# uthree/ALiVE-VC

Measured on AMD Instinct MI355X. Metric: VC frames/sec + RTF @24kHz, 1M-vec library; 1/2/4/8 MI355X, higher is better.
Workload: dtype decoder fp16 GEMMs / fp32 acc; encoders 22-bit fp16 split; kNN exact fp32 top-k via fp6 MFMA candidates (certified); f32 MFMA small convs; f64 phase scan

## Files before the change

### alive-vc_amd/csrc/conv.hip

```cpp
#include "conv_epilogue.h"
#include "planes_layout.h"

namespace {

constexpr int BK = 16;
constexpr int A_LD = BK + 4;

template <int BM, int BN, int WM, int WN, bool UPV = false, bool YPL = false>
__global__ __launch_bounds__(256) void conv_gemm_kernel(AliveConv p, unsigned kw_magic, unsigned kw_shift, float film_ratio) {
    constexpr int TM = BM / WM, TN = BN / WN;
    constexpr int MR = TM / 16, NR = TN / 16;
    constexpr int B_LD = BN + 4;
    constexpr int ROWS_PER_PASS = 256 / BN;
    constexpr int EPT = BK / ROWS_PER_PASS;
    constexpr int A_VEC = (BM * 4 + 255) / 256;
    static_assert(WM * WN == 4, "4 waves");
    static_assert(256 % BN == 0 || BN == 256, "BN");

    __shared__ __attribute__((aligned(16))) float As[2][BM][A_LD];
    __shared__ __attribute__((aligned(16))) float Bs[2][BK][B_LD];

    const int tid = threadIdx.x;
    const int lane = tid & 63;
    const int wid = tid >> 6;
// ... 117 lines not shown
                if (p.up == 4) {
                    if (row < p.Co) *(f32x4*)(p.Y + ((size_t)n * Cq + (row >> 2)) * Lout + (size_t)t * 4) = acc[m][nn];
                } else {
#pragma unroll
                    for (int h = 0; h < 2; ++h)
                        if (row + 2 * h < p.Co) {
                            f32x2 v = {acc[m][nn][2 * h], acc[m][nn][2 * h + 1]};
                            *(f32x2*)(p.Y + ((size_t)n * Cq + (row >> 1) + h) * Lout + (size_t)t * 2) = v;
                        }
                }
            }
        }
        return;
    }
#pragma unroll
    for (int nn = 0; nn < NR; ++nn) {
        const int t = t0 + wn * TN + nn * 16 + lr;
        if (t >= p.Tout) continue;
        Lerp lp;
        if (p.Z != nullptr) lp = lerp_coord(t, film_ratio, p.Lf);
#pragma unroll
        for (int m = 0; m < MR; ++m) {
#pragma unroll
            for (int r = 0; r < 4; ++r) {
                const int row_local = wm * TM + m * 16 + lq * 4 + r;
                if (m0 + row_local >= p.Co) continue;
                conv_epilogue_store<false>(p, n, m0 + row_local, row_local, t, acc[m][nn][r], lp, ft);
            }
        }
        if constexpr (YPL) {
            static_assert(!YPL || (MR % 2) == 0, "the plane image pairs the 16-row groups");
            const int c_pad = (p.Co + 31) & ~31;
            const int64_t cols_pad = (((int64_t)p.N * p.Tout + 127) / 128) * 128;
            unsigned short* Po = (unsigned short*)p.Yp;
            const bool odd = (lq & 1) != 0;
#pragma unroll
            for (int mp = 0; mp < MR; mp += 2) {
                const int rbase = m0 + wm * TM + mp * 16;
                if (rbase >= c_pad) continue;
                float qa[4], qb[4];
#pragma unroll
                for (int r = 0; r < 4; ++r) {
                    qa[r] = rbase + lq * 4 < p.Co ? acc[mp][nn][r] : 0.0f;
                    qb[r] = rbase + 16 + lq * 4 < p.Co ? acc[mp + 1][nn][r] : 0.0f;
                }
                const bool one_f16 = p.yp_planes == 1;
#pragma unroll
                for (int pl = 0; pl < 2; ++pl) {
                    if (pl == 1 && one_f16) break;
                    typedef __bf16 bf16x2_t __attribute__((ext_vector_type(2)));
                    auto pk = [one_f16](float a, float b) {
                        const bf16x2_t h = {(__bf16)a, (__bf16)b};
                        return one_f16 ? pack_f16x2(a, b) : __builtin_bit_cast(unsigned, h);
                    };
                    const unsigned a01 = pk(qa[0], qa[1]), a23 = pk(qa[2], qa[3]), b01 = pk(qb[0], qb[1]), b23 = pk(qb[2], qb[3]);
                    const unsigned rx = (unsigned)__shfl_xor((int)(odd ? a01 : b01), 16), ry = (unsigned)__shfl_xor((int)(odd ? a23 : b23), 16);
                    const u32x4 o = odd ? u32x4{rx, ry, b01, b23} : u32x4{a01, a23, rx, ry};
                    const int ch = rbase + (odd ? 16 + (lq - 1) * 4 : lq * 4);
                    *(u32x4*)(Po + planes_at(pl, (int64_t)n * p.Tout + t, ch, cols_pad, c_pad)) = o;
                    qa[0] -= __uint_as_float(a01 << 16); qa[1] -= __uint_as_float(a01 & 0xffff0000u);
                    qa[2] -= __uint_as_float(a23 << 16); qa[3] -= __uint_as_float(a23 & 0xffff0000u);
                    qb[0] -= __uint_as_float(b01 << 16); qb[1] -= __uint_as_float(b01 & 0xffff0000u);
                    qb[2] -= __uint_as_float(b23 << 16); qb[3] -= __uint_as_float(b23 & 0xffff0000u);
                }
            }
        }
    }
    if constexpr (YPL) {
        if (n == p.N - 1 && blockIdx.x == gridDim.x - 1) {
            const int c_pad = (p.Co + 31) & ~31;
            const int64_t cols = (int64_t)p.N * p.Tout, cols_pad = ((cols + 127) / 128) * 128;
            const int per_col = (p.yp_planes == 1 ? 1 : 2) * (c_pad / 4);
            unsigned short* Po = (unsigned short*)p.Yp;
            for (int i = threadIdx.x; i < (int)(cols_pad - cols) * per_col; i += 256) {
                const int c = i / per_col, w = i % per_col;
                *(uint2*)(Po + planes_at(w / (c_pad / 4), cols + c, (w % (c_pad / 4)) * 4, cols_pad, c_pad)) = make_uint2(0u, 0u);
            }
        }
    }
}

}

int alive_conv_split_launch(const AliveConv* d, float ratio, hipStream_t s);
bool alive_conv_skinny_try(const AliveConv* d, hipStream_t s, int* rc);

extern "C" int alive_conv1d(const AliveConv* d, void* stream) {
    ALIVE_CHECK_ARG(d && d->W && (d->X || d->Xp), "alive_conv1d: null W/X");
    ALIVE_CHECK_ARG(d->N > 0 && d->Ci > 0 && d->Co > 0 && d->Tin > 0 && d->Tout > 0, "alive_conv1d: bad sizes");
    ALIVE_CHECK_ARG(d->KW >= 1 && (d->KW <= 16 || d->Ci == 1) && d->stride >= 1 && d->dil >= 1 && d->up >= 1, "alive_conv1d: bad geometry");
    ALIVE_CHECK_ARG(d->precision >= 1 || (d->K_pad % 16 == 0 && d->K_pad >= d->Ci * d->KW), "alive_conv1d: K_pad %d for K %d", d->K_pad, d->Ci * d->KW);
    ALIVE_CHECK_ARG(d->precision >= 0 && d->precision <= 3, "alive_conv1d: precision");
    ALIVE_CHECK_ARG(d->Ci * d->KW < 32768, "alive_conv1d: K too large");
    ALIVE_CHECK_ARG(d->Y || d->Z || d->Zp, "alive_conv1d: no output");
    if (d->up > 1) {
        ALIVE_CHECK_ARG(d->Co % d->up == 0 && !d->residual && !d->skip && !d->Z && !d->Zp && d->Y, "alive_conv1d: transposed conv has a plain epilogue");
    }
    ALIVE_CHECK_ARG(d->yp_planes >= 0 && d->yp_planes <= 2, "alive_conv1d: yp_planes");
    if (d->Yp)
        ALIVE_CHECK_ARG(d->precision == 0 && d->Y && d->up == 1 && d->act == 0 && !d->post_add && !d->ch_scale && !d->residual && !d->skip && !d->Z &&
                        !d->Zp && d->Co > 16 && d->Co <= 64 && (d->Co & 3) == 0 && (((uintptr_t)d->Yp) & 15) == 0 && (int64_t)d->N * d->Tout >= 97,
                        "alive_conv1d: Yp (plane image of Y) needs the exact kernel's plain conv with 16 < Co <= 64, Co %% 4 == 0, more than 96 columns");
    ALIVE_CHECK_ARG(d->pad_mode >= 0 && d->pad_mode <= 2, "alive_conv1d: pad_mode");
    if (d->pad_mode != 0) ALIVE_CHECK_ARG(d->pad_left < d->Tin, "alive_conv1d: reflect pad %d needs Tin > pad (Tin %d)", d->pad_left, d->Tin);
    if (d->Z || d->Zp) ALIVE_CHECK_ARG(d->film && d->Lf > 0, "alive_conv1d: Z needs film");
    ALIVE_CHECK_ARG(d->film_ld != 0 || (d->film_t0 == 0 && d->film_f0 == 0), "alive_conv1d: film_t0 %d / film_f0 %d without a frame range (film_ld 0)",
                    d->film_t0, d->film_f0);
    if (d->precision == 3)
        ALIVE_CHECK_ARG((int64_t)d->N * d->Tout > 96, "alive_conv1d: precision 3 (plain fp16) is a batch form: more than 96 columns, got %lld",
                        (long long)d->N * d->Tout);
    if (d->Xp || d->Zp) ALIVE_CHECK_ARG(d->precision == 1 || d->precision == 3, "alive_conv1d: plane-packed operands need the split kernel (precision 1 or 3)");
    {
        int rc;
        if (d->film_ld == 0 && !d->Xp && !d->Zp && alive_conv_skinny_try(d, (hipStream_t)stream, &rc)) return rc;
    }
    if (d->precision >= 1)
        return alive_conv_split_launch(d, (d->Z || d->Zp) ? (float)(d->film_ld ? d->film_ld : d->Lf) / (float)d->Tout : 0.0f, (hipStream_t)stream);
    ALIVE_CHECK_ARG(d->film_ld == 0, "alive_conv1d: a film frame range needs the split kernel (precision 1 / 2)");
    const unsigned shift = d->KW < 4 ? 18u : d->KW < 8 ? 19u : 20u;
    const unsigned magic = d->Ci == 1 ? 0u : (unsigned)(((1u << shift) + d->KW - 1) / d->KW);
    const float ratio = d->Z ? (float)d->Lf / (float)d->Tout : 0.0f;
    hipStream_t s = (hipStream_t)stream;
    if (d->Co > 64) {
        dim3 g(cdiv(d->Tout, 128), cdiv(d->Co, 128), d->N);
        conv_gemm_kernel<128, 128, 2, 2><<<g, 256, 0, s>>>(*d, magic, shift, ratio);
    } else if (d->Co > 16) {
        dim3 g(cdiv(d->Tout, 128), cdiv(d->Co, 64), d->N);
        if (d->Yp) conv_gemm_kernel<64, 128, 1, 4, false, true><<<g, 256, 0, s>>>(*d, magic, shift, ratio);
        else conv_gemm_kernel<64, 128, 1, 4><<<g, 256, 0, s>>>(*d, magic, shift, ratio);
    } else {
        dim3 g(cdiv(d->Tout, 256), 1, d->N);
        if ((d->up == 2 || d->up == 4) && d->act == 0 && !d->post_add && !d->ch_scale)
            conv_gemm_kernel<16, 256, 1, 4, true><<<g, 256, 0, s>>>(*d, magic, shift, ratio);
        else
            conv_gemm_kernel<16, 256, 1, 4><<<g, 256, 0, s>>>(*d, magic, shift, ratio);
    }
    ALIVE_CHECK_LAUNCH("alive_conv1d");
    return ALIVE_OK;
}

ALIVE_F16_SAT_GETTER(alive_f16_sat_conv)
```

### alive-vc_amd/csrc/conv_split.hip

```cpp
#include "conv_epilogue.h"
#include "planes_layout.h"

namespace {

constexpr int BN = 128;
constexpr int BKC = 32;
constexpr int XROWS = 144;
constexpr int PITCH = 80;
constexpr int XPLANE = XROWS * PITCH;

typedef __bf16 bf16x2_t __attribute__((ext_vector_type(2)));

__device__ __forceinline__ bf16x8 lds_frag(const unsigned char* p) { return *(const bf16x8*)p; }

typedef const __attribute__((address_space(1))) void* gptr_t;
typedef __attribute__((address_space(3))) void* lptr_t;
constexpr int PROW = 64;

template <int BM, int NP, bool PLANES = false, bool W22 = false>
__global__ __launch_bounds__(256, 2) void conv_split_kernel(AliveConv p, float film_ratio) {
    static_assert(!W22 || BM == 128, "the 2 x 2 wave arrangement is the 128-row tile's");
    constexpr int NR = W22 ? 2 : (BM >= 128 ? 4 : 2);
    constexpr int MR = W22 ? 2 : 1;

// ... 302 lines not shown
            }
        } else if (upvec) {
            const int sh = __builtin_ctz((unsigned)p.up);
            const size_t Lout = (size_t)p.Tout * p.up;
#pragma unroll
            for (int g = tid; g < PR * (BN / 4); g += 256) {
                const int e = g * 4;
                const int co_l = e >> (7 + sh), rem = e & ((BN << sh) - 1);
                const int t_l = rem >> sh, j0 = rem & (p.up - 1);
                const int pr = (co_l << sh) + j0;
                const int row = m0 + ps * 64 + pr;
                const int t = t0 + t_l;
                if (row >= p.Co || t >= p.Tout) continue;
                f32x4 v;
#pragma unroll
                for (int q = 0; q < 4; ++q) {
                    float x = Ct[(pr + q) * CP + t_l];
                    if (p.act == 1) x = gelu_fast(x);
                    else if (p.act == 2) x = expf(x);
                    if (p.post_add != nullptr) x += p.post_add[row + q];
                    if (p.ch_scale != nullptr) x *= p.ch_scale[row + q];
                    v[q] = x;
                }
                *(f32x4*)(p.Y + ((size_t)n * (p.Co >> sh) + (row >> sh)) * Lout + ((size_t)t << sh) + j0) = v;
            }
        } else if (p.up > 1) {
            const unsigned inv_up = (unsigned)((0x100000000ull + (unsigned)p.up - 1) / (unsigned)p.up);
            const int R0 = m0 + ps * 64;
            const int c_first = (int)__umulhi((unsigned)R0, inv_up);
            int R1 = R0 + PR - 1;
            R1 = R1 < p.Co ? R1 : p.Co - 1;
            const int nch = (int)__umulhi((unsigned)R1, inv_up) - c_first + 1;
            const int per_ch = BN * p.up;
            const size_t Lout = (size_t)p.Tout * p.up;
            const int Cq = (int)__umulhi((unsigned)p.Co, inv_up);
#pragma unroll 1
            for (int ch = 0; ch < nch; ++ch) {
                const int co = c_first + ch;
                float* yrow = p.Y + ((size_t)n * Cq + co) * Lout + (size_t)t0 * p.up;
#pragma unroll 2
                for (int e = tid; e < per_ch; e += 256) {
                    const int t_l = (int)__umulhi((unsigned)e, inv_up), jj = e - t_l * p.up;
                    const int row = co * p.up + jj;
                    if (row < R0 || row > R1 || t0 + t_l >= p.Tout) continue;
                    float v = Ct[(row - R0) * CP + t_l];
                    if (p.act == 1) v = gelu_fast(v);
                    else if (p.act == 2) v = expf(v);
                    if (p.post_add != nullptr) v = v + p.post_add[row];
                    if (p.ch_scale != nullptr) v = v * p.ch_scale[row];
                    yrow[e] = v;
                }
            }
        } else {
#pragma unroll 1
            for (int g = tid; g < PR * BN; g += 256) {
                const int pr = g >> 7, c = g & 127;
                const int row = m0 + ps * 64 + pr;
                const int t = t0 + c;
                if (row >= p.Co || t >= p.Tout) continue;
                float v = Ct[pr * CP + c];
                if (p.act == 1) v = gelu_fast(v);
                else if (p.act == 2) v = expf(v);
                if (p.post_add != nullptr) v = v + p.post_add[row];
                if (p.ch_scale != nullptr) v = v * p.ch_scale[row];
                const size_t o = ((size_t)n * p.Co + row) * p.Tout + t;
                if (p.residual != nullptr) v = v + p.residual[o];
                if (p.skip != nullptr) v = v + p.skip[o];
                if (p.Y != nullptr) p.Y[o] = v;
                if (p.Z != nullptr) {
                    const float* fs = Ft + pr * 2 * FILM_NF - f_lo;
                    Lerp lp = lerp_coord(t + p.film_t0, film_ratio, p.Lf);
                    float sc = lerp_apply(lp, fs[lp.i0], fs[lp.i1]);
                    float sh = lerp_apply(lp, fs[FILM_NF + lp.i0], fs[FILM_NF + lp.i1]);
                    p.Z[o] = gelu_fast(v) * sc + sh;
                }
            }
        }
        __syncthreads();
    }
}

}

int alive_conv_split_launch(const AliveConv* d, float ratio, hipStream_t s) {
    ALIVE_CHECK_ARG(d->stride == 1, "alive_conv1d(split): stride must be 1");
    ALIVE_CHECK_ARG(d->Ci_pad % BKC == 0 && d->Ci_pad >= d->Ci, "alive_conv1d(split): Ci_pad %d for Ci %d", d->Ci_pad, d->Ci);
    ALIVE_CHECK_ARG(d->KW <= 8 && (d->KW - 1) * d->dil <= XROWS - BN, "alive_conv1d(split): halo (KW-1)*dil = %d exceeds %d",
                    (d->KW - 1) * d->dil, XROWS - BN);
    ALIVE_CHECK_ARG(d->pad_mode == 0 || d->pad_mode == 1, "alive_conv1d(split): pad_mode");
    ALIVE_CHECK_ARG(((((uintptr_t)d->Y) | ((uintptr_t)d->Z) | ((uintptr_t)d->residual) | ((uintptr_t)d->skip)) & 15) == 0,
                    "alive_conv1d(split): Y / Z / residual / skip must be 16-byte aligned");
    if (d->Z) {
        const double span = (double)(d->film_ld ? d->film_ld : d->Lf) / (double)d->Tout * BN + 3.0;
        ALIVE_CHECK_ARG(span <= FILM_NF, "alive_conv1d(split): FiLM second output needs Tout >= ~8 Lf (got Lf %d, Tout %d)", d->Lf, d->Tout);
    }
    ALIVE_CHECK_ARG(d->act >= 0 && d->act <= 2, "alive_conv1d(split): activation %d not available on the split kernel", d->act);
    if (d->Zp) {
        const double span = (double)(d->film_ld ? d->film_ld : d->Lf) / (double)d->Tout * BN + 3.0;
        ALIVE_CHECK_ARG(span <= FILM_NF && d->film, "alive_conv1d(split): plane second output needs FiLM rows and Tout >= ~8 Lf");
        ALIVE_CHECK_ARG(d->up == 1 && (d->Tout & 3) == 0 && d->Co % 64 == 0 && d->Co > 64 && (d->precision == 1 || d->precision == 3) &&
                        (((uintptr_t)d->Zp) & 15) == 0,
                        "alive_conv1d(split): plane second output needs up 1, Tout %% 4 == 0, Co a multiple of 64 above 64, precision 1 or 3");
    }
    if (d->Xp) {
        ALIVE_CHECK_ARG((d->precision == 1 || d->precision == 3) && d->Co > 64 && d->Ci % BKC == 0 && d->Ci_pad == d->Ci && (d->pad_mode == 1 || d->pad_left == 0) &&
                        (((uintptr_t)d->Xp) & 15) == 0 && d->Tout <= d->Tin &&
                        (int64_t)(d->Tout - 1) * d->stride + (int64_t)(d->KW - 1) * d->dil - d->pad_left < d->Tin,
                        "alive_conv1d(split): plane input needs precision 1 or 3, Co > 64, Ci a multiple of 32, reflect-left padding and no valid "
                        "output column that reads past the signal (the kernel clamps rows >= Tin instead of zero-filling them)");
    }
    ALIVE_CHECK_ARG(d->Tout <= d->Tin + d->pad_left, "alive_conv1d(split): Tout");
    if (d->precision == 3) {
        if (d->Co > 64) {
            dim3 g(cdiv(d->Tout, BN), cdiv(d->Co, 128), d->N);
            if (d->Xp) conv_split_kernel<128, 1, true, true><<<g, 256, 0, s>>>(*d, ratio);
            else conv_split_kernel<128, 1, false, true><<<g, 256, 0, s>>>(*d, ratio);
        } else {
            dim3 g(cdiv(d->Tout, BN), 1, d->N);
            conv_split_kernel<64, 1><<<g, 256, 0, s>>>(*d, ratio);
        }
    } else if (d->Co > 64) {
        dim3 g(cdiv(d->Tout, BN), cdiv(d->Co, 128), d->N);
        if (d->precision == 2) conv_split_kernel<128, 3><<<g, 256, 0, s>>>(*d, ratio);
        else if (d->Xp) conv_split_kernel<128, 2, true><<<g, 256, 0, s>>>(*d, ratio);
        else conv_split_kernel<128, 2><<<g, 256, 0, s>>>(*d, ratio);
    } else {
        dim3 g(cdiv(d->Tout, BN), 1, d->N);
        if (d->precision == 2) conv_split_kernel<64, 3><<<g, 256, 0, s>>>(*d, ratio);
        else conv_split_kernel<64, 2><<<g, 256, 0, s>>>(*d, ratio);
    }
    ALIVE_CHECK_LAUNCH("alive_conv1d(split)");
    return ALIVE_OK;
}

ALIVE_F16_SAT_GETTER(alive_f16_sat_conv_split)
```

### alive-vc_amd/module/_native.py

```python
import ctypes as C
import os

import torch

_HERE = os.path.dirname(os.path.abspath(__file__))
LIB_PATH = os.environ.get("ALIVE_VC_LIB", os.path.join(os.path.dirname(_HERE), "libalive_vc.so"))

_lib = None


class AliveConv(C.Structure):
    _fields_ = [
        ("W", C.c_void_p), ("bias", C.c_void_p), ("X", C.c_void_p),
        ("N", C.c_int), ("Ci", C.c_int), ("Tin", C.c_int), ("Co", C.c_int), ("K_pad", C.c_int),
        ("KW", C.c_int), ("stride", C.c_int), ("dil", C.c_int), ("pad_left", C.c_int), ("pad_mode", C.c_int),
        ("Tout", C.c_int), ("up", C.c_int), ("act", C.c_int),
        ("post_add", C.c_void_p), ("ch_scale", C.c_void_p), ("residual", C.c_void_p), ("skip", C.c_void_p),
        ("Y", C.c_void_p), ("Z", C.c_void_p), ("film", C.c_void_p),
        ("film_rows", C.c_int), ("Lf", C.c_int), ("film_scale_row", C.c_int), ("film_shift_row", C.c_int),
        ("precision", C.c_int), ("Ci_pad", C.c_int),
        ("film_t0", C.c_int), ("film_f0", C.c_int), ("film_ld", C.c_int),
        ("Xp", C.c_void_p), ("Zp", C.c_void_p), ("Yp", C.c_void_p), ("yp_planes", C.c_int),
    ]


class AliveGemm(C.Structure):
    _fields_ = [
        ("W", C.c_void_p), ("bias", C.c_void_p), ("P", C.c_void_p),
        ("N", C.c_int), ("T", C.c_int), ("Ci", C.c_int), ("Co", C.c_int), ("planes", C.c_int), ("act", C.c_int),
        ("post_add", C.c_void_p), ("ch_scale", C.c_void_p), ("residual", C.c_void_p),
        ("Y", C.c_void_p), ("Pout", C.c_void_p),
        ("b_plane", C.c_int64), ("b_win", C.c_int64), ("b_row", C.c_int), ("b_cblk", C.c_int), ("b_blk", C.c_int64),
        ("arg_val", C.c_void_p), ("arg_idx", C.c_void_p),
        ("Y2", C.c_void_p), ("y_split", C.c_int),
        ("f16s", C.c_int), ("wscale", C.c_void_p), ("in_unscale", C.c_float), ("pout_scale", C.c_float),
    ]


_VP, _I, _I64, _F, _D, _SZ = C.c_void_p, C.c_int, C.c_int64, C.c_float, C.c_double, C.c_size_t

PROTOTYPES = {
    "alive_last_error": (C.c_char_p, []),
    "alive_version": (_I, []),
    "alive_library_padded_rows": (_I64, [_I64]),
    "alive_library_pack": (_I, [_VP, _I64, _I, _VP, _VP, _VP, _VP]),
    "alive_knn_workspace_bytes": (_SZ, [_I64, _I64]),
    "alive_knn_workspace_bytes_strict": (_SZ, [_I64, _I64]),
    "alive_knn_workspace_bytes_fast": (_SZ, [_I64, _I64]),
    "alive_knn_search": (_I, [_VP, _I, _I, _VP, _VP, _VP, _I64, _I64, _I, _VP, _VP, _VP, _VP]),
    "alive_library_fp8_bytes": (_SZ, [_I64]),
    "alive_library_rounding_bound": (_I, [_VP, _VP, _VP, _I64, _VP, _VP]),
    "alive_library_pack_lo": (_I, [_VP, _VP, _VP, _I64, _VP, _VP]),
    "alive_knn_search_strict": (_I, [_VP, _I, _I, _VP, _VP, _VP, _VP, _VP, _I64, _I64, _I, _VP, _VP, _VP, _VP, _VP, _VP]),
    "alive_library_pack_fp8": (_I, [_VP, _I64, _VP, _VP]),
    "alive_knn_search_fp8": (_I, [_VP, _I, _I, _VP, _VP, _VP, _VP, _I64, _I64, _I, _VP, _VP, _VP, _VP]),
    "alive_knn_search_stats": (_VP, [_I, _I, _I64, _VP]),
    "alive_debug_knn_stage_view": (_I, [_I64, _I64, _I, _I, _VP, _I]),
    "alive_knn_search_timed": (_I, [_VP, _I, _I, _VP, _VP, _VP, _I64, _I64, _I, _VP, _VP, _VP, _VP, _VP, _VP]),
    "alive_knn_search_fp8_timed": (_I, [_VP, _I, _I, _VP, _VP, _VP, _VP, _I64, _I64, _I, _VP, _VP, _VP, _VP, _VP, _VP]),
    "alive_library_pack_fp6": (_I, [_VP, _I64, _VP, _VP]),
    "alive_knn_sub_coordinates": (_I, []),
    "alive_knn_workspace_bytes_sub": (_SZ, [_I64, _I64]),
    "alive_library_fp6_sub_bytes": (_SZ, [_I64]),
    "alive_library_pack_fp6_sub": (_I, [_VP, _I64, _I64, _I64, _VP, _VP, _VP, _VP]),
    "alive_knn_search_fp6_sub_timed": (_I, [_VP, _VP, _I, _I, _VP, _VP, _VP, _VP, _VP, _VP, _I64, _I64, _I, _VP, _VP, _VP, _VP, _VP, _VP]),
    "alive_knn_rot_coordinates": (_I, []),
    "alive_knn_rot_leading": (_I, []),
    "alive_knn_rot_mixed": (_I, []),
    "alive_library_pack_fp8_rot": (_I, [_VP, _I64, _I64, _I64, _F, _VP, _VP]),
    "alive_knn_search_fp8_rot_timed": (_I, [_VP, _VP, _F, _I, _I, _VP, _VP, _VP, _VP, _I64, _I64, _I, _VP, _VP, _VP, _VP, _VP, _VP]),
    "alive_knn_search_fp6": (_I, [_VP, _I, _I, _VP, _VP, _VP, _VP, _I64, _I64, _I, _VP, _VP, _VP, _VP]),
    "alive_knn_search_fp6_timed": (_I, [_VP, _I, _I, _VP, _VP, _VP, _VP, _I64, _I64, _I, _VP, _VP, _VP, _VP, _VP, _VP]),
    "alive_library_pack_rows": (_I, [_VP, _I64, _I, _VP, _VP, _VP]),
    "alive_knn_grouped_workspace_bytes": (_SZ, [_I, _I, _I]),
    "alive_knn_search_grouped": (_I, [_VP, _I, _I, _VP, _VP, _I64, _VP, _VP, _I, _VP, _VP, _VP, _VP]),
    "alive_knn_merge_gather_rows": (_I, [_VP, _VP, _I, _VP, _VP, _VP, _I, _I, _VP, _VP, _VP]),
    "alive_knn_blend_gather_rows": (_I, [_VP, _VP, _I, _VP, _VP, _VP, _VP, _VP, _I, _I, _VP, _VP]),
    "alive_knn_grouped_k_workspace_bytes": (_SZ, [_I, _I, _I]),
    "alive_knn_search_grouped_k": (_I, [_VP, _I, _I, _VP, _VP, _I64, _VP, _VP, _VP, _I, _VP, _VP, _VP, _VP]),
    "alive_knn_merge_gather_rows_k": (_I, [_VP, _VP, _VP, _I, _VP, _VP, _VP, _I, _I, _VP, _VP, _VP]),
    "alive_knn_blend_gather_rows_k": (_I, [_VP, _VP, _VP, _I, _VP, _VP, _VP, _VP, _VP, _I, _I, _VP, _VP]),
    "alive_pool_append": (_I, [_VP, _I64, _I64, _I64, _I, _VP, _VP, _I64, _I64, _VP, _VP]),
    "alive_pool_move_rows": (_I, [_VP, _VP, _I64, _I64, _I64, _I64, _VP]),
    "alive_pool_image_bytes": (_SZ, [_VP, _I, _VP]),
    "alive_pool_pack_images": (_I, [_VP, _VP, _I64, _VP, _VP, _I, _VP, _VP, _VP]),
    "alive_knn_pool_workspace_bytes": (_SZ, [_I, _I, _I, _I, _I64, _I64]),
    "alive_knn_search_pool": (_I, [_VP, _I, _I, _VP, _VP, _VP, _VP, _VP, _I64, _VP, _VP, _I, _I64, _VP, _I, _VP, _VP, _VP, _VP]),
    "alive_knn_pool_k_workspace_bytes": (_SZ, [_I, _I, _I, _I, _I64, _I64]),
    "alive_knn_search_pool_k": (_I, [_VP, _I, _I, _VP, _VP, _VP, _VP, _VP, _I64, _VP, _VP, _I, _I64, _VP, _VP, _I, _VP, _VP, _VP, _VP]),
    "alive_knn_pool_stats": (_VP, [_VP]),
    "alive_dedup_pass": (_I, [_VP, _VP, _I64, _I, _D, _VP, _VP, _VP]),
    "alive_knn_merge_gather": (_I, [_VP, _VP, _I, _I, _D, _VP, _VP, _I, _I, _VP, _VP, _VP]),
    "alive_conv1d": (_I, [C.POINTER(AliveConv), _VP]),
    "alive_decoder_precision": (_I, [_I]),
    "alive_encoder_precision": (_I, [_I]),
    "alive_f16_saturations": (_I, [_I]),
    "alive_f16_saturations_clear": (_I, [_VP]),
    "alive_gelu_film": (_I, [_VP, _I, _I, _I, _VP, _I, _I, _I, _I, _I, _I, _I, _VP, _VP, _VP]),
    "alive_planes_bytes": (_SZ, [_I64, _I, _I]),
    "alive_to_planes": (_I, [_VP, _I, _I, _I, _I, _VP, _VP]),
    "alive_gemm_planes": (_I, [C.POINTER(AliveGemm), _VP]),
    "alive_argmax_merge": (_I, [_VP, _VP, _I, _I64, _VP, _VP]),
    "alive_filter_block_small_weights": (_I, [_I]),
    "alive_filter_block_small": (_I, [_VP, _I, _I, _I, _VP, _VP, _I, _I, _I, _VP, _VP, _VP]),
    "alive_filter_block_small_range": (_I, [_VP, _I, _I, _I, _VP, _VP, _I, _I, _I, _I, _I, _I, _VP, _VP, _VP]),
    "alive_filter_block_small_up_range": (_I, [_VP, _I, _I, _VP, _VP, _I, _I, _I, _I, _I, _I, _VP, _VP, _VP, _VP, _VP]),
    "alive_filter_block_small_wave_range": (_I, [_VP, _I, _I, _VP, _VP, _I, _I, _I, _I, _I, _I, _VP, _VP, _VP, _VP]),
    "alive_filter_block64_weights": (_I64, []),
    "alive_filter_block64": (_I, [_VP, _I, _I, _VP, _VP, _VP, _I, _I, _I, _VP, _VP, _VP]),
    "alive_filter_block64_range": (_I, [_VP, _I, _I, _VP, _VP, _VP, _I, _I, _I, _I, _I, _I, _VP, _VP, _VP]),
    "alive_filter_block64_range_fp16": (_I, [_VP, _I, _I, _VP, _VP, _VP, _I, _I, _I, _I, _I, _I, _VP, _VP, _VP]),
    "alive_filter_block256_workspace_bytes": (_I64, [_I, _I]),
    "alive_filter_block256_fp16": (_I, [_VP, _I, _I, _VP, _VP, _VP, _I, _I, _I, _I, _I, _I, _VP, _VP, _VP, _I64, _VP]),
    "alive_filter_block64s_workspace_bytes": (_I64, [_I, _I]),
    "alive_filter_block64s_fp16": (_I, [_VP, _I, _I, _VP, _VP, _VP, _I, _I, _I, _I, _I, _I, _VP, _VP, _VP, _I64, _VP]),
    "alive_filter_block64s_fp16_up": (_I, [_VP, _I, _I, _VP, _VP, _VP, _I, _I, _I, _I, _I, _I, _VP, _VP, _VP, _VP, _VP, _I64, _VP]),
    "alive_filter_source_in": (_I, [_VP, _I, _I, _VP, _VP, _VP, _VP, _VP, _VP]),
    "alive_filter_source_out": (_I, [_VP, _I, _I, _VP, _VP, _VP, _VP]),
    "alive_dwconv_norm": (_I, [_VP, _I, _I, _I, _VP, _VP, _I, _VP, _VP, _VP, _I, _I, _I, _F, _VP, _VP]),
    "alive_dwconv_norm_planes": (_I, [_VP, _I, _I, _I, _VP, _VP, _I, _VP, _VP, _VP, _I, _I, _I, _F, _I, _VP, _VP]),
    "alive_dwconv_norm_planes_f16s": (_I, [_VP, _I, _I, _I, _VP, _VP, _I, _VP, _VP, _VP, _I, _I, _I, _F, _F, _VP, _VP]),
    "alive_dwconv_norm_planes_ref": (_I, [_VP, _I, _I, _I, _VP, _VP, _I, _VP, _VP, _VP, _I, _I, _I, _F, _I, _VP, _VP, _F]),
    "alive_channel_norm": (_I, [_VP, _I, _I, _I, _VP, _VP, _F, _VP, _VP]),
    "alive_argmax_channels": (_I, [_VP, _I, _I, _I, _VP, _VP]),
    "alive_oscillator_workspace_bytes": (_SZ, [_I, _I, _I]),
    "alive_oscillator": (_I, [_VP, _VP, _VP, _I, _I, _I, _I, _F, _I, _I, _VP, _VP, _VP, _VP]),
    "alive_oscillator_range": (_I, [_VP, _VP, _VP, _I, _I, _I, _I, _F, _I, _I, _I, _I, _VP, _VP, _VP, _VP]),
    "alive_dft_basis_bytes": (_SZ, []),
    "alive_dft_basis": (_I, [_VP, _VP]),
    "alive_spectrogram_workspace_bytes": (_SZ, [_I, _I]),
    "alive_spectrogram": (_I, [_VP, _VP, _I, _I, _VP, _VP, _VP]),
    "alive_resample_taps": (_I, [_I, _I]),
    "alive_resample_length": (_I64, [_I64, _I, _I]),
    "alive_resample_filter": (_I, [_I, _I, _VP, _VP]),
    "alive_resample": (_I, [_VP, _I, _I, _I, _I, _VP, _F, _F, _VP, _I, _VP]),
    "alive_resample_rows": (_I, [_VP, _I, _I, _I, _I, _VP, _VP, _VP, _VP, _I, _VP]),
    "alive_resample_rows_multi": (_I, [_VP, _I, _I, _VP, _VP, _VP, _I, _VP, _I64, _I, _VP, _VP, _VP, _I, _VP, _VP]),
    "alive_pcm16_to_float": (_I, [_VP, _I64, _VP, _VP]),
    "alive_float_to_pcm16": (_I, [_VP, _I64, _VP, _VP]),
    "alive_weight_count": (_I, [_I]),
    "alive_weight_name": (C.c_char_p, [_I, _I]),
    "alive_front_end_workspace_bytes": (_SZ, [_I, _I]),
    "alive_front_end": (_I, [_VP, _VP, _VP, _VP, _VP, _VP, _I, _I, _VP, _VP, _VP, _VP]),
    "alive_content_encoder_workspace_bytes": (_SZ, [_I, _I]),
    "alive_content_encoder": (_I, [_VP, _VP, _I, _I, _VP, _VP, _VP]),
    "alive_f0_estimate_workspace_bytes": (_SZ, [_I, _I]),
    "alive_f0_estimate": (_I, [_VP, _VP, _I, _I, _VP, _VP, _VP]),
    "alive_f0_logits": (_I, [_VP, _VP, _I, _I, _VP, _VP, _VP]),
    "alive_f0_track_workspace_bytes": (_SZ, [_I, _I, _I]),
    "alive_f0_track_rows": (_I, [_VP, _I, _I, _I, _I, _I, _VP, _VP, _VP, _VP, _VP, _VP, _VP, _VP, _VP, _VP]),
    "alive_decoder_workspace_bytes": (_SZ, [_I, _I]),
    "alive_decoder_forward": (_I, [_VP, _VP, _VP, _VP, _I, _I, _I, _I, _VP, _VP, _VP, _VP]),
    "alive_decoder_forward_range": (_I, [_VP, _VP, _VP, _I, _I, _I, _I, _VP, _VP, _VP]),
    "alive_pitch_transform": (_I, [_VP, _I, _I, _I, _F, _F, _F, _VP]),
    "alive_pitch_transform_rows": (_I, [_VP, _I, _I, _I, _VP, _VP, _VP, _VP]),
    "alive_pitch_stats_groups": (_I, [_VP, _I, _I, _I, _I, _VP, _I, _VP, _VP]),
    "alive_pitch_shift_groups": (_I, [_VP, _VP, _I, _I, _VP, _VP, _VP, _VP, _VP]),
    "alive_pitch_follow_rows": (_I, [_VP, _I, _I, _VP, _VP, _VP, _VP, _VP, _D, _D, _VP, _VP, _VP]),
    "alive_pitch_stats2_groups": (_I, [_VP, _I, _I, _I, _I, _VP, _I, _VP, _VP]),
    "alive_pitch_range_groups": (_I, [_VP, _VP, _I, _I, _VP, _VP, _VP, _D, _VP, _VP, _VP, _VP]),
    "alive_pitch_follow2_rows": (_I, [_VP, _I, _I, _VP, _VP, _VP, _VP, _VP, _VP, _VP, _VP, _D, _D, _D, _VP, _VP, _VP, _VP, _VP, _VP]),
    "alive_pitch_transform_rows_centred": (_I, [_VP, _I, _I, _I, _VP, _VP, _VP, _VP, _VP, _VP]),
    "alive_gate_rows": (_I, [_VP, _I, _I, _I, _I, _VP, _VP, _VP, _VP, _VP, _I, _VP, _VP, _VP, _VP, _VP, _VP, _VP, _VP, _VP]),
    "alive_gate_apply_rows": (_I, [_VP, _I, _I, _VP, _VP, _VP, _VP, _VP]),
    "alive_seam_rows": (_I, [_VP, _I, _I, _VP, _VP, _VP, _VP, _VP, _VP, _VP, _I, _VP, _VP, _VP]),
    "alive_limit_rows": (_I, [_VP, _I, _I, _VP, _VP, _VP, _VP, _VP, _VP, _VP, _VP, _I, _VP, _VP]),
    "alive_limit_waves": (_I, [_VP, _VP, _I, _I, _VP, _I, _I, _VP, _VP, _VP]),
    "alive_loudness_workspace_bytes": (_SZ, [_I, _I]),
    "alive_loudness_measure_waves": (_I, [_VP, _I, _I, _VP, _VP, _VP, _VP, _D, _I, _VP, _VP, _VP, _VP, _SZ, _VP]),
    "alive_loudness_apply_waves": (_I, [_VP, _VP, _I, _I, _VP, _VP, _VP, _VP, _D, _VP, _VP]),
    "alive_loudness_rows": (_I, [_VP, _I, _I, _VP, _VP, _VP, _VP, _VP, _VP, _VP, _VP, _VP]),
    "alive_envelope_waves": (_I,[_VP, _VP, _I, _VP, _I, _I, _VP, _VP, _I, _I, _D, _D, _D, _VP, _VP]),
    "alive_ring_push_rows": (_I, [_VP, _I, _I, _VP, _I, _VP, _VP, _VP, _VP, _I, _I, _VP, _VP, _VP, _VP, _VP]),
    "alive_emit_rows": (_I, [_VP, _I, _I, _VP, _VP, _VP, _VP, _I, _VP]),
    "alive_conceal_rows": (_I, [_VP, _I, _I, _VP, _VP, _I, _VP, _VP, _VP, _VP, _VP, _VP, _VP, _VP, _VP, _VP, _VP, _VP, _I, _VP]),
    "alive_codebook_workspace_bytes": (_SZ, [_I64, _I64]),
# ... 84 lines not shown
```

### include/alive_vc.h

```cpp
#ifndef ALIVE_VC_H
#define ALIVE_VC_H

#include <stddef.h>
#include <stdint.h>

#ifdef __cplusplus
extern "C" {
#endif

#define ALIVE_OK 0
#define ALIVE_ERR_ARG (-1)
#define ALIVE_ERR_LAUNCH (-2)

#define ALIVE_DIM 768
#define ALIVE_KPRIME 16
#define ALIVE_MAX_K 64

const char* alive_last_error(void);
int alive_version(void);

int64_t alive_library_padded_rows(int64_t M);
int alive_library_pack(const float* tokens_DxM, int64_t M, int D,
                       void* lib_bf16, float* rows_f32, float* norms, void* stream);

// ... 60 lines not shown
                                   int64_t idx_base, int k, float* out_val, int32_t* out_idx, void* ws, void* stream,
                                   void* ev_start, void* ev_stop);

int alive_knn_merge_gather(const float* cand_val, const int32_t* cand_idx, int n_shards, int k,
                           double alpha, const float* rows_f32_full, const float* src,
                           int N, int T, float* out, int32_t* final_idx, void* stream);

int alive_library_pack_rows(const float* tokens, int64_t M, int Dd, float* rows_f32, float* norms, void* stream);
size_t alive_knn_grouped_workspace_bytes(int N, int T, int k);
int alive_knn_search_grouped(const float* src, int N, int T, const float* rows_f32, const float* norms, int64_t P,
                             const int32_t* seg_lo, const int32_t* seg_len, int k, float* out_val, int32_t* out_idx,
                             void* ws, void* stream);
int alive_knn_merge_gather_rows(const float* cand_val, const int32_t* cand_idx, int k, const double* alpha,
                                const float* rows_f32_full, const float* src, int N, int T, float* out,
                                int32_t* final_idx, void* stream);
#define ALIVE_MAX_BLEND 4
int alive_knn_blend_gather_rows(const float* cand_val, const int32_t* cand_idx, int k, const int32_t* first,
                                const double* weight, const double* alpha, const float* rows_f32_full, const float* src,
                                int N, int T, float* out, void* stream);

size_t alive_knn_grouped_k_workspace_bytes(int N, int T, int k_max);
int alive_knn_search_grouped_k(const float* src, int N, int T, const float* rows_f32, const float* norms, int64_t P,
                               const int32_t* seg_lo, const int32_t* seg_len, const int32_t* k_row, int k_max, float* out_val,
                               int32_t* out_idx, void* ws, void* stream);
int alive_knn_merge_gather_rows_k(const float* cand_val, const int32_t* cand_idx, const int32_t* k_row, int k_max,
                                  const double* alpha, const float* rows_f32_full, const float* src, int N, int T, float* out,
                                  int32_t* final_idx, void* stream);
int alive_knn_blend_gather_rows_k(const float* cand_val, const int32_t* cand_idx, const int32_t* k_row, int k_max,
                                  const int32_t* first, const double* weight, const double* alpha, const float* rows_f32_full,
                                  const float* src, int N, int T, float* out, void* stream);

int alive_pool_append(const float* tokens, int64_t row_stride, int64_t col_stride, int64_t M, int Dd, float* rows_f32,
                      float* norms, int64_t capacity, int64_t at, int32_t* report, void* stream);
int alive_pool_move_rows(float* rows_f32, float* norms, int64_t capacity, int64_t src, int64_t dst, int64_t n, void* stream);

#define ALIVE_POOL_STATS 8
size_t alive_pool_image_bytes(const int32_t* seg_len, int V, int64_t* img_off);
int alive_pool_pack_images(const float* rows_f32, const float* norms, int64_t P, const int32_t* seg_lo, const int32_t* seg_len,
                           int V, void* images, float* bounds, void* stream);
size_t alive_knn_pool_workspace_bytes(int N, int T, int k, int V, int64_t P, int64_t max_len);
int alive_knn_search_pool(const float* src, int N, int T, const void* images, const int64_t* img_off, const float* rows_f32,
                          const float* norms, const float* bounds, int64_t P, const int32_t* seg_lo, const int32_t* seg_len,
                          int V, int64_t max_len, const int32_t* voice, int k, float* out_val, int32_t* out_idx, void* ws,
                          void* stream);
size_t alive_knn_pool_k_workspace_bytes(int N, int T, int k_max, int V, int64_t P, int64_t max_len);
int alive_knn_search_pool_k(const float* src, int N, int T, const void* images, const int64_t* img_off, const float* rows_f32,
                            const float* norms, const float* bounds, int64_t P, const int32_t* seg_lo, const int32_t* seg_len,
                            int V, int64_t max_len, const int32_t* voice, const int32_t* k_row, int k_max, float* out_val,
                            int32_t* out_idx, void* ws, void* stream);
const int* alive_knn_pool_stats(void* ws);

int alive_dedup_pass(const float* val, const int32_t* idx, int64_t M, int k, double threshold, int32_t* state,
                     int32_t* undecided, void* stream);

typedef struct AliveConv {
    const float* W;
    const float* bias;
    const float* X;
    int N, Ci, Tin;
    int Co;
    int K_pad;
    int KW, stride, dil;
    int pad_left;
    int pad_mode;
    int Tout;
    int up;
    int act;
    const float* post_add;
    const float* ch_scale;
    const float* residual;
    const float* skip;
    float* Y;
    float* Z;
    const float* film;
    int film_rows, Lf, film_scale_row, film_shift_row;
    int precision, Ci_pad;
    int film_t0, film_f0, film_ld;
    const void* Xp;
    void* Zp;
    void* Yp;
    int yp_planes;
} AliveConv;
int alive_conv1d(const AliveConv* desc, void* stream);

size_t alive_planes_bytes(int64_t cols, int C, int planes);
int alive_to_planes(const float* X, int N, int C, int T, int planes, void* P, void* stream);
typedef struct AliveGemm {
    const void* W;
    const float* bias;
    const void* P;
    int N, T;
    int Ci, Co;
    int planes;
    int act;
    const float* post_add;
    const float* ch_scale;
    const float* residual;
    float* Y;
    void* Pout;
    int64_t b_plane, b_win;
    int b_row;
    int b_cblk;
    int64_t b_blk;
    float* arg_val;
    int32_t* arg_idx;
    float* Y2;
    int y_split;
    int f16s;
    const float* wscale;
    float in_unscale, pout_scale;
} AliveGemm;
int alive_gemm_planes(const AliveGemm* desc, void* stream);
int alive_argmax_merge(const float* arg_val, const int32_t* arg_idx, int nblk, int64_t cols, float* out, void* stream);

int alive_filter_block_small_weights(int C);
int alive_filter_block_small(const float* U, int N, int C, int L, const float* wpack, const float* film,
                             int film_rows, int Lf, int film_off, const float* skip, float* out, void* stream);
int alive_filter_block_small_range(const float* U, int N, int C, int L, const float* wpack, const float* film,
                                   int film_rows, int Lf, int film_off, int t0, int f0, int film_ld, const float* skip,
                                   float* out, void* stream);
int alive_filter_block_small_up_range(const float* U, int N, int L, const float* wpack, const float* film, int film_rows, int Lf,
                                      int film_off, int t0, int f0, int film_ld, const float* skip, const float* upW, const float* upb,
                                      float* out, void* stream);
int alive_filter_block_small_wave_range(const float* U, int N, int L, const float* wpack, const float* film, int film_rows, int Lf,
                                        int film_off, int t0, int f0, int film_ld, const float* oW, const float* ob, float* wave,
                                        void* stream);

int64_t alive_filter_block64_weights(void);
int alive_filter_block64(const float* U, int N, int L, const void* W16, const float* biases, const float* film,
                         int film_rows, int Lf, int film_off, const float* skip, float* out, void* stream);
int alive_filter_block64_range(const float* U, int N, int L, const void* W16, const float* biases, const float* film,
                               int film_rows, int Lf, int film_off, int t0, int f0, int film_ld, const float* skip,
                               float* out, void* stream);
int alive_filter_block64_range_fp16(const float* U, int N, int L, const void* W16, const float* biases, const float* film,
                               int film_rows, int Lf, int film_off, int t0, int f0, int film_ld, const float* skip,
                               float* out, void* stream);

int64_t alive_filter_block256_workspace_bytes(int N, int L);
int alive_filter_block256_fp16(const float* U, int N, int L, const void* const* w16, const float* const* bias, const float* film,
                               int film_rows, int Lf, int film_off, int t0, int f0, int film_ld, const float* skip, float* out,
                               void* ws, int64_t ws_bytes, void* stream);

int64_t alive_filter_block64s_workspace_bytes(int N, int L);
int alive_filter_block64s_fp16(const float* U, int N, int L, const void* const* w16, const float* const* bias, const float* film,
                               int film_rows, int Lf, int film_off, int t0, int f0, int film_ld, const float* skip, float* out,
                               void* ws, int64_t ws_bytes, void* stream);
int alive_filter_block64s_fp16_up(const float* U, int N, int L, const void* const* w16, const float* const* bias, const float* film,
                                  int film_rows, int Lf, int film_off, int t0, int f0, int film_ld, const float* skip, const float* upW,
                                  const float* upb, float* out, void* ws, int64_t ws_bytes, void* stream);

int alive_filter_source_in(const float* src, int N, int Lw, const float* Win, const float* bin, const float* Wd,
                           const float* bd, float* d0, void* stream);
int alive_filter_source_out(const float* H, int N, int Lw, const float* W, const float* b, float* wave, void* stream);

int alive_dwconv_norm(const float* X, int N, int C, int T, const float* dw_w, const float* dw_b,
                      int affine_mode, const float* gain, const float* offset,
                      const float* cond, int cond_rows, int scale_row, int shift_row,
                      float eps, float* Y, void* stream);
int alive_dwconv_norm_planes(const float* X, int N, int C, int T, const float* dw_w, const float* dw_b,
                             int affine_mode, const float* gain, const float* offset,
                             const float* cond, int cond_rows, int scale_row, int shift_row,
                             float eps, int planes, void* P, void* stream);
int alive_dwconv_norm_planes_f16s(const float* X, int N, int C, int T, const float* dw_w, const float* dw_b,
                                  int affine_mode, const float* gain, const float* offset,
                                  const float* cond, int cond_rows, int scale_row, int shift_row,
                                  float eps, float scale, void* P, void* stream);
// ... 160 lines not shown
```

Baseline: 1.350 million.

## Add dedicated pointwise transposed-conv kernel for split-precision upsampling layers

Adds a specialized MFMA kernel for KW=1 transposed (up>1) convolutions in the split bf16 precision path. It stages the whole input tile in LDS once as hi/lo bf16 planes, then walks all output-channel tiles per wave with a ring of prefetched weight fragments, scattering results directly into the interleaved upsampled layout. It is meant to avoid the generic split kernel's per-tile re-splitting of the input and its poor fit for the upsample shape. It only engages above a minimum block count, and the old tiled path stays reachable through a new entry point.

```diff
diff --git a/alive-vc_amd/csrc/conv.hip b/alive-vc_amd/csrc/conv.hip
--- a/alive-vc_amd/csrc/conv.hip
+++ b/alive-vc_amd/csrc/conv.hip
@@ -223,10 +223,10 @@
 
 }
 
-int alive_conv_split_launch(const AliveConv* d, float ratio, hipStream_t s);
+int alive_conv_split_launch(const AliveConv* d, float ratio, hipStream_t s, bool allow_up);
 bool alive_conv_skinny_try(const AliveConv* d, hipStream_t s, int* rc);
 
-extern "C" int alive_conv1d(const AliveConv* d, void* stream) {
+static int conv1d_impl(const AliveConv* d, void* stream, bool allow_up) {
     ALIVE_CHECK_ARG(d && d->W && (d->X || d->Xp), "alive_conv1d: null W/X");
     ALIVE_CHECK_ARG(d->N > 0 && d->Ci > 0 && d->Co > 0 && d->Tin > 0 && d->Tout > 0, "alive_conv1d: bad sizes");
     ALIVE_CHECK_ARG(d->KW >= 1 && (d->KW <= 16 || d->Ci == 1) && d->stride >= 1 && d->dil >= 1 && d->up >= 1, "alive_conv1d: bad geometry");
@@ -256,7 +256,8 @@
         if (d->film_ld == 0 && !d->Xp && !d->Zp && alive_conv_skinny_try(d, (hipStream_t)stream, &rc)) return rc;
     }
     if (d->precision >= 1)
-        return alive_conv_split_launch(d, (d->Z || d->Zp) ? (float)(d->film_ld ? d->film_ld : d->Lf) / (float)d->Tout : 0.0f, (hipStream_t)stream);
+        return alive_conv_split_launch(d, (d->Z || d->Zp) ? (float)(d->film_ld ? d->film_ld : d->Lf) / (float)d->Tout : 0.0f, (hipStream_t)stream,
+                                       allow_up);
     ALIVE_CHECK_ARG(d->film_ld == 0, "alive_conv1d: a film frame range needs the split kernel (precision 1 / 2)");
     const unsigned shift = d->KW < 4 ? 18u : d->KW < 8 ? 19u : 20u;
     const unsigned magic = d->Ci == 1 ? 0u : (unsigned)(((1u << shift) + d->KW - 1) / d->KW);
@@ -280,4 +281,7 @@
     return ALIVE_OK;
 }
 
+extern "C" int alive_conv1d(const AliveConv* d, void* stream) { return conv1d_impl(d, stream, true); }
+extern "C" int alive_conv1d_tiled(const AliveConv* d, void* stream) { return conv1d_impl(d, stream, false); }
+
 ALIVE_F16_SAT_GETTER(alive_f16_sat_conv)
diff --git a/alive-vc_amd/csrc/conv_split.hip b/alive-vc_amd/csrc/conv_split.hip
--- a/alive-vc_amd/csrc/conv_split.hip
+++ b/alive-vc_amd/csrc/conv_split.hip
@@ -408,7 +408,9 @@
 
 }
 
-int alive_conv_split_launch(const AliveConv* d, float ratio, hipStream_t s) {
+bool alive_conv_up_try(const AliveConv* d, hipStream_t s, int* rc);
+
+int alive_conv_split_launch(const AliveConv* d, float ratio, hipStream_t s, bool allow_up) {
     ALIVE_CHECK_ARG(d->stride == 1, "alive_conv1d(split): stride must be 1");
     ALIVE_CHECK_ARG(d->Ci_pad % BKC == 0 && d->Ci_pad >= d->Ci, "alive_conv1d(split): Ci_pad %d for Ci %d", d->Ci_pad, d->Ci);
     ALIVE_CHECK_ARG(d->KW <= 8 && (d->KW - 1) * d->dil <= XROWS - BN, "alive_conv1d(split): halo (KW-1)*dil = %d exceeds %d",
@@ -436,6 +438,10 @@
                         "output column that reads past the signal (the kernel clamps rows >= Tin instead of zero-filling them)");
     }
     ALIVE_CHECK_ARG(d->Tout <= d->Tin + d->pad_left, "alive_conv1d(split): Tout");
+    {
+        int rc;
+        if (allow_up && alive_conv_up_try(d, s, &rc)) return rc;
+    }
     if (d->precision == 3) {
         if (d->Co > 64) {
             dim3 g(cdiv(d->Tout, BN), cdiv(d->Co, 128), d->N);
diff --git a/alive-vc_amd/csrc/conv_up.hip b/alive-vc_amd/csrc/conv_up.hip
--- /dev/null
+++ b/alive-vc_amd/csrc/conv_up.hip
@@ -0,0 +1,235 @@
+#include <atomic>
+#include <type_traits>
+#include "common.h"
+#include "planes_layout.h"
+
+namespace {
+
+constexpr int UBN = 64;
+constexpr int UKC = 32;
+constexpr int UCI_MAX = 256;
+constexpr int UROW = 64;
+constexpr int UCB = UBN * UROW;
+constexpr int UPLANE = (UCI_MAX / UKC) * UCB;
+constexpr int UP_MIN_BLOCKS = 512;
+std::atomic<int> g_up_min_blocks{UP_MIN_BLOCKS};
+
+typedef __bf16 bf16x2_t __attribute__((ext_vector_type(2)));
+typedef float f32x2 __attribute__((ext_vector_type(2)));
+
+std::atomic<int> g_up_launches{0};
+
+template <int ST, int NCB>
+__global__ __launch_bounds__(256, 2) void conv_up_kernel(AliveConv p, unsigned inv_up) {
+    __shared__ __attribute__((aligned(16))) unsigned char smem[2 * UPLANE];
+
+    const int tid = threadIdx.x, lane = tid & 63, wid = tid >> 6;
+    const int lr = lane & 31, lh = lane >> 5;
+    const int n = blockIdx.y, t0 = blockIdx.x * UBN;
+    const int co_pad = (p.Co + 15) & ~15;
+    const int ncb = p.Ci / UKC;
+    const int ntile = (p.Co + 31) >> 5;
+    const unsigned short* W16 = (const unsigned short*)p.W;
+    const size_t wplane = (size_t)p.Ci * co_pad;
+
+    auto fetch = [&](int tile, int cb, bf16x8 (&a)[2][2]) {
+        if (tile < ntile) {
+            int grow = tile * 32 + lr;
+            grow = grow < co_pad ? grow : co_pad - 1;
+            const unsigned short* w = W16 + ((size_t)cb * co_pad + grow) * PLANES_KB + lh * 8;
+#pragma unroll
+            for (int s2 = 0; s2 < 2; ++s2)
+#pragma unroll
+                for (int pl = 0; pl < 2; ++pl) a[s2][pl] = *(const bf16x8*)(w + pl * wplane + s2 * 16);
+        }
+    };
+    constexpr int RING = NCB == 8 ? 4 : 1;
+    bf16x8 a_ring[RING][2][2];
+    if constexpr (NCB == 8) {
+#pragma unroll
+        for (int cb = 0; cb < 3; ++cb) fetch(wid, cb, a_ring[cb]);
+    }
+
+    {
+        const int tcol = t0 + lane;
+        const bool ok = tcol < p.Tin;
+        const float* Xl = p.X + ((size_t)n * p.Ci + wid * 8) * p.Tin + (ok ? tcol : p.Tin - 1);
+        unsigned char* dst = smem + lane * UROW + ((wid ^ ((lane >> 2) & 3)) << 4);
+        for (int cb0 = 0; cb0 < ncb; cb0 += 4) {
+            float x[4][8];
+#pragma unroll
+            for (int u = 0; u < 4; ++u)
+                if (cb0 + u < ncb) {
+#pragma unroll
+                    for (int c = 0; c < 8; ++c) x[u][c] = Xl[(size_t)((cb0 + u) * UKC + c) * p.Tin];
+                }
+#pragma unroll
+            for (int u = 0; u < 4; ++u)
+                if (cb0 + u < ncb) {
+                    u32x4 hv, lv;
+#pragma unroll
+                    for (int e = 0; e < 4; ++e) {
+                        const float x0 = ok ? x[u][2 * e] : 0.0f, x1 = ok ? x[u][2 * e + 1] : 0.0f;
+                        bf16x2_t hp = {(__bf16)x0, (__bf16)x1};
+                        const unsigned h = __builtin_bit_cast(unsigned, hp);
+                        const float r0 = x0 - __uint_as_float(h << 16), r1 = x1 - __uint_as_float(h & 0xffff0000u);
+                        bf16x2_t lp = {(__bf16)r0, (__bf16)r1};
+                        hv[e] = h;
+                        lv[e] = __builtin_bit_cast(unsigned, lp);
+                    }
+                    *(u32x4*)(dst + (cb0 + u) * UCB) = hv;
+                    *(u32x4*)(dst + (cb0 + u) * UCB + UPLANE) = lv;
+                }
+        }
+    }
+    __syncthreads();
+
+    const unsigned char* bbase = smem + lr * UROW;
+    const int bsw0 = ((0 + lh) ^ ((lr >> 2) & 3)) << 4, bsw1 = ((2 + lh) ^ ((lr >> 2) & 3)) << 4;
+    auto load_B = [&](int cb, int s2, bf16x8 (&b)[2][2]) {
+        const unsigned char* q = bbase + cb * UCB + (s2 ? bsw1 : bsw0);
+#pragma unroll
+        for (int pl = 0; pl < 2; ++pl)
+#pragma unroll
+            for (int nn = 0; nn < 2; ++nn) b[pl][nn] = *(const bf16x8*)(q + pl * UPLANE + nn * 32 * UROW);
+    };
+    auto load_bias = [&](int tile, f32x16& raw) {
+        if (p.bias != nullptr) {
+#pragma unroll
+            for (int r = 0; r < 16; ++r) {
+                const int row = tile * 32 + (r & 3) + 8 * (r >> 2) + 4 * lh;
+                raw[r] = p.bias[row < p.Co ? row : p.Co - 1];
+            }
+        }
+    };
+
+    const size_t Lout = (size_t)p.Tout * p.up;
+    float* Yn = p.Y + (size_t)n * (p.Co / p.up) * Lout;
+    auto walk = [&](auto two_c) {
+        constexpr bool TWO = decltype(two_c)::value;
+        constexpr int NR = TWO ? 2 : 1;
+        f32x16 acc[NR];
+        auto mfma6 = [&](const bf16x8 (&a)[2], const bf16x8 (&b)[2][2]) {
+#pragma unroll
+            for (int nn = 0; nn < NR; ++nn) {
+                acc[nn] = __builtin_amdgcn_mfma_f32_32x32x16_bf16(a[0], b[1][nn], acc[nn], 0, 0, 0);
+                acc[nn] = __builtin_amdgcn_mfma_f32_32x32x16_bf16(a[1], b[0][nn], acc[nn], 0, 0, 0);
+                acc[nn] = __builtin_amdgcn_mfma_f32_32x32x16_bf16(a[0], b[0][nn], acc[nn], 0, 0, 0);
+            }
+        };
+        bf16x8 b0[2][2], b1[2][2];
+        f32x16 bias_raw;
+#pragma unroll
+        for (int r = 0; r < 16; ++r) bias_raw[r] = 0.0f;
+        load_bias(wid, bias_raw);
+        load_B(0, 0, b0);
+        for (int tile = wid; tile < ntile; tile += 4) {
+#pragma unroll
+            for (int r = 0; r < 16; ++r) {
+                const int row = tile * 32 + (r & 3) + 8 * (r >> 2) + 4 * lh;
+                const float v = row < p.Co ? bias_raw[r] : 0.0f;
+#pragma unroll
+                for (int nn = 0; nn < NR; ++nn) acc[nn][r] = v;
+            }
+            if (tile + 4 < ntile) load_bias(tile + 4, bias_raw);
+            auto step = [&](int cb, const bf16x8 (&a)[2][2]) {
+                load_B(cb, 1, b1);
+                mfma6(a[0], b0);
+                load_B(cb + 1 < ncb ? cb + 1 : 0, 0, b0);
+                mfma6(a[1], b1);
+            };
+            if constexpr (NCB == 8) {
+#pragma unroll
+                for (int cb = 0; cb < 8; ++cb) {
+                    fetch(cb + 3 < 8 ? tile : tile + 4, (cb + 3) & 7, a_ring[(cb + 3) & 3]);
+                    step(cb, a_ring[cb & 3]);
+                }
+            } else {
+                for (int cb = 0; cb < ncb; ++cb) {
+                    fetch(tile, cb, a_ring[0]);
+                    step(cb, a_ring[0]);
+                }
+            }
+            __builtin_amdgcn_sched_barrier(0);
+#pragma unroll
+            for (int nn = 0; nn < NR; ++nn) {
+                const int t = t0 + nn * 32 + lr;
+                if (t >= p.Tout) continue;
+                float* yt = Yn + (size_t)t * p.up;
+#pragma unroll
+                for (int q = 0; q < 4; ++q) {
+                    const int R0 = tile * 32 + 8 * q + 4 * lh;
+                    if (ST == 0) {
+                        if (R0 < p.Co) {
+                            const int co = (int)__umulhi((unsigned)R0, inv_up), j = R0 - co * p.up;
+                            *(f32x4*)(yt + (size_t)co * Lout + j) = f32x4{acc[nn][4 * q], acc[nn][4 * q + 1], acc[nn][4 * q + 2], acc[nn][4 * q + 3]};
+                        }
+                    } else if (ST == 1) {
+#pragma unroll
+                        for (int h = 0; h < 2; ++h) {
+                            const int R = R0 + 2 * h;
+                            if (R < p.Co) {
+                                const int co = (int)__umulhi((unsigned)R, inv_up), j = R - co * p.up;
+                                *(f32x2*)(yt + (size_t)co * Lout + j) = f32x2{acc[nn][4 * q + 2 * h], acc[nn][4 * q + 2 * h + 1]};
+                            }
+                        }
+                    } else {
+#pragma unroll
+                        for (int h = 0; h < 4; ++h) {
+                            const int R = R0 + h;
+                            if (R < p.Co) {
+                                const int co = (int)__umulhi((unsigned)R, inv_up), j = R - co * p.up;
+                                yt[(size_t)co * Lout + j] = acc[nn][4 * q + h];
+                            }
+                        }
+                    }
+                }
+            }
+            __builtin_amdgcn_sched_barrier(0);
+        }
+    };
+    if (p.Tout - t0 > 32) walk(std::true_type{});
+    else walk(std::false_type{});
+}
+
+}
+
+bool alive_conv_up_try(const AliveConv* d, hipStream_t s, int* rc) {
+    if (d->precision != 1 || d->KW != 1 || d->stride != 1 || d->up <= 1 || d->pad_left != 0) return false;
+    if (d->Ci % UKC != 0 || d->Ci != d->Ci_pad || d->Ci > UCI_MAX) return false;
+    if (d->act != 0 || d->post_add || d->ch_scale || d->residual || d->skip || d->Z || d->Zp || d->Xp || !d->X || !d->Y) return false;
+    if (d->Co % d->up != 0 || d->Co > (1 << 24) || d->Tout > d->Tin || d->N > 65535) return false;
+    const int64_t tiles = cdiv(d->Tout, UBN);
+    if ((int64_t)d->N * tiles < g_up_min_blocks.load(std::memory_order_relaxed)) return false;
+    const unsigned inv_up = (unsigned)((0x100000000ull + (unsigned)d->up - 1) / (unsigned)d->up);
+    dim3 g((unsigned)tiles, (unsigned)d->N);
+    const int st = d->up % 4 == 0 ? 0 : d->up % 2 == 0 ? 1 : 2;
+    if (d->Ci == 8 * UKC) {
+        if (st == 0) conv_up_kernel<0, 8><<<g, 256, 0, s>>>(*d, inv_up);
+        else if (st == 1) conv_up_kernel<1, 8><<<g, 256, 0, s>>>(*d, inv_up);
+        else conv_up_kernel<2, 8><<<g, 256, 0, s>>>(*d, inv_up);
+    } else {
+        if (st == 0) conv_up_kernel<0, 0><<<g, 256, 0, s>>>(*d, inv_up);
+        else if (st == 1) conv_up_kernel<1, 0><<<g, 256, 0, s>>>(*d, inv_up);
+        else conv_up_kernel<2, 0><<<g, 256, 0, s>>>(*d, inv_up);
+    }
+    g_up_launches.fetch_add(1, std::memory_order_relaxed);
+    hipError_t e = hipGetLastError();
+    if (e != hipSuccess) {
+        alive_set_error("alive_conv1d(up): %s", hipGetErrorString(e));
+        *rc = ALIVE_ERR_LAUNCH;
+    } else {
+        *rc = ALIVE_OK;
+    }
+    return true;
+}
+
+extern "C" int alive_conv_up_min_blocks(int blocks) {
+    if (blocks > 0) g_up_min_blocks.store(blocks, std::memory_order_relaxed);
+    else if (blocks < 0) g_up_min_blocks.store(UP_MIN_BLOCKS, std::memory_order_relaxed);
+    return g_up_min_blocks.load(std::memory_order_relaxed);
+}
+
+extern "C" int alive_conv_up_launches(int reset) {
+    return reset ? g_up_launches.exchange(0, std::memory_order_relaxed) : g_up_launches.load(std::memory_order_relaxed);
+}
diff --git a/alive-vc_amd/module/_native.py b/alive-vc_amd/module/_native.py
--- a/alive-vc_amd/module/_native.py
+++ b/alive-vc_amd/module/_native.py
@@ -92,6 +92,9 @@
     "alive_dedup_pass": (_I, [_VP, _VP, _I64, _I, _D, _VP, _VP, _VP]),
     "alive_knn_merge_gather": (_I, [_VP, _VP, _I, _I, _D, _VP, _VP, _I, _I, _VP, _VP, _VP]),
     "alive_conv1d": (_I, [C.POINTER(AliveConv), _VP]),
+    "alive_conv1d_tiled": (_I, [C.POINTER(AliveConv), _VP]),
+    "alive_conv_up_launches": (_I, [_I]),
+    "alive_conv_up_min_blocks": (_I, [_I]),
     "alive_decoder_precision": (_I, [_I]),
     "alive_encoder_precision": (_I, [_I]),
     "alive_f16_saturations": (_I, [_I]),
diff --git a/include/alive_vc.h b/include/alive_vc.h
--- a/include/alive_vc.h
+++ b/include/alive_vc.h
@@ -166,6 +166,9 @@
     int yp_planes;
 } AliveConv;
 int alive_conv1d(const AliveConv* desc, void* stream);
+int alive_conv1d_tiled(const AliveConv* desc, void* stream);
+int alive_conv_up_launches(int reset);
+int alive_conv_up_min_blocks(int blocks);
 
 size_t alive_planes_bytes(int64_t cols, int C, int planes);
 int alive_to_planes(const float* X, int N, int C, int T, int planes, void* P, void* stream);
```

Result: faster. 1.378 million (median of 6 runs) (+2.1%).
